# google-deepmind/meltingpot

Hardware: NVIDIA H100
Metric: env_steps_per_sec (higher is better)
Workload: dtype u8

## Files before the change

meltingpot_b200/build.py:

```python

from __future__ import annotations

import os
import shutil
import subprocess

_HERE = os.path.dirname(os.path.abspath(__file__))
SOURCES = ['engine.cu']
HEADERS = ['common.cuh', 'family_load.h', 'render.cuh', 'step_common.cuh', 'step_clean_up.cuh', 'step_commons.cuh', 'step_territory.cuh', 'step_coins.cuh', 'step_mining.cuh', 'state_bank.cuh']
LIB_PATH = os.path.join(_HERE, 'libmpengine.so')

NVCC_FLAGS = [
    '-gencode', 'arch=compute_90a,code=sm_90a', '-lineinfo', '-O3',
    '-std=c++17', '--fmad=false', '-shared', '-Xcompiler', '-fPIC',
]


def _nvcc() -> str:
  for cand in (shutil.which('nvcc'), '/usr/local/cuda/bin/nvcc'):
    if cand and os.path.exists(cand):
      return cand
  raise FileNotFoundError('nvcc not found')


def is_stale() -> bool:
  if not os.path.exists(LIB_PATH):
    return True
  built = os.path.getmtime(LIB_PATH)
  deps = [os.path.join(_HERE, 'csrc', f) for f in SOURCES + HEADERS]
  root = os.path.dirname(_HERE)
  deps += [os.path.join(root, 'include', 'mp_engine.h'),
           os.path.join(root, 'include', 'mpb_format.h')]
  return any(os.path.getmtime(d) > built for d in deps if os.path.exists(d))


def build(force: bool = False, verbose: bool = False) -> str:
  if not force and not is_stale():
    return LIB_PATH
  cmd = [_nvcc()] + NVCC_FLAGS
  if verbose:
    cmd += ['-Xptxas', '-v']
  cmd += ['-o', LIB_PATH] + [os.path.join(_HERE, 'csrc', s) for s in SOURCES]
  subprocess.check_call(cmd)
  return LIB_PATH


if __name__ == '__main__':
  print(build(force=True, verbose=True))
```

meltingpot_b200/csrc/engine.cu:

```cuda
#include <cuda_runtime.h>

#include <algorithm>
#include <cstdio>
#include <cstring>
#include <map>
#include <string>
#include <variant>
#include <vector>

#include "../../include/mp_engine.h"
#include "../../include/mpb_format.h"
#include "common.cuh"
#include "family_load.h"
#include "render.cuh"
#include "step_clean_up.cuh"
#include "step_commons.cuh"
#include "step_territory.cuh"
#include "step_coins.cuh"
#include "step_mining.cuh"
#include "state_bank.cuh"

static_assert(MP_MAX_ROUTE_CHOICES == MP_ROUTE_CHOICES && MP_MAX_ROUTE_PLAYERS == MP_MAX_PLAYERS,
              "mp_route_draw's table is DrawnActions'");
namespace {
// ... 825 lines not shown
  RecordLayout& R = E->record;
  R = RecordLayout{};
  uint32_t off = 16;
  int rc = MP_OK;
  auto row = [&](void* base, uint32_t bytes, uint32_t align) {
    if (R.n_rows == MP_RECORD_MAX_ROWS) { rc = fail(MP_E_UNSUPPORTED, "more than %d per-env state arrays", MP_RECORD_MAX_ROWS); return; }
    off = (off + align - 1) / align * align;
    R.row[R.n_rows++] = {static_cast<uint8_t*>(base), bytes, bytes, off};
    off += bytes;
  };
  auto own = [&](auto*& p, uint32_t bytes, uint32_t align = 16) {
    if (allocate && !rc) rc = E->alloc((size_t)E->B * bytes / sizeof *p, &p);
    row(p, bytes, align);
  };
  own(S.key, 8, 8);
  row(E->variants.active, 1, 1); row(E->variants.pending, 1, 1);
  own(S.grid, T.L * T.cells_pad * 2); own(S.avatar, P * 16); own(S.av_timer, P * 16);
  own(S.apple, T.nA_pad); own(S.dirt, T.nD_pad); own(S.water, T.nW_pad); own(S.apple_count, T.nA_pad);
  own(S.fam_u8, S.fam_u8_stride); own(S.fam_u16, S.fam_u16_stride * 2); own(S.av_extra, P * 32);
  own(S.packed, (P + 2) * 8); own(S.env, ENV_COLS * 4);
  row(S.reward, P * 8, 16); row(S.discount, 8, 16); row(S.step_type, 8, 16);
  for (int k = 0; k < T.n_scalar; ++k) row(S.scalar_obs + (size_t)k * E->B * P, P * 8, 16);
  own(S.events, S.max_events * 12); own(S.n_events, 4);
  if (rc) return rc;
  R.record_bytes = (off + 15) / 16 * 16;
  const uint64_t h = E->blob_hash;
  R.tag = make_uint4(kRecordFormat, (uint32_t)R.record_bytes, (uint32_t)h, (uint32_t)(h >> 32));
  CUDA_TRY(cudaMemcpy(E->d_record_layout, &R, sizeof R, cudaMemcpyHostToDevice));
  return MP_OK;
}

}

extern "C" {

const char* mp_last_error(void) { return g_error.c_str(); }
const char* mp_version(void) { return "meltingpot_b200 engine 0.1 (sm_90a)"; }

}

namespace {
int setup_variants(Decoded& D, const void* const* blobs, const size_t* blob_bytes, int n);
int upload_tables(mp_engine* E, Decoded& D);
int upload_variants(mp_engine* E, const Decoded& D, const void* const* blobs, const size_t* blob_bytes, int n, const uint8_t* env_variant_host);

int create(const void* const* blobs, const size_t* blob_sizes, int n_blobs, const uint8_t* env_variant, int num_envs, int device,
           uint64_t seed, uint64_t env_index_base, uint32_t flags, mp_handle* out) {
  Decoded D(n_blobs);
  int rc = build_tables(D, blobs, blob_sizes, n_blobs, flags);
  if (rc == MP_OK && n_blobs > 1) rc = setup_variants(D, blobs, blob_sizes, n_blobs);
  if (rc != MP_OK) return rc;
  int n_dev = 0;
  cudaError_t e = cudaGetDeviceCount(&n_dev);
  if (e != cudaSuccess || n_dev == 0) return fail(MP_E_NO_DEVICE, "no CUDA device available (%s); this engine has no CPU path", cudaGetErrorString(e));
  if (device < 0 || device >= n_dev || device >= MP_MAX_DEVICES) return fail(MP_E_INVALID, "device %d out of range (0..%d)", device, n_dev - 1);
  cudaDeviceProp prop;
  CUDA_TRY(cudaGetDeviceProperties(&prop, device));
  if (prop.major != 9 || prop.minor != 0) return fail(MP_E_NO_DEVICE, "device %d is sm_%d%d; kernels are built for sm_90a only", device, prop.major, prop.minor);
  DeviceGuard guard(device);
  mp_engine* E = new mp_engine();
  clear_last_launch(E);
  E->device = device; E->B = num_envs; E->flags = flags; E->sm_count = prop.multiProcessorCount;
  E->blob_hash = fnv1a(blobs[0], blob_sizes[0]);
  rc = upload_tables(E, D);
  if (rc == MP_OK && n_blobs > 1) rc = upload_variants(E, D, blobs, blob_sizes, n_blobs, env_variant);
  if (rc == MP_OK) rc = build_plan(E);
  if (rc != MP_OK) {
    const std::string msg = g_error;
    mp_destroy(E);
    g_error = msg;
    return rc;
  }
  const Tables& T = E->T;
  State& S = E->S;
  S.B = num_envs; E->key_base = seed + env_index_base;
  const size_t B = num_envs, P = T.P;
  {
    S.max_events = round_up(std::max(MP_MIN_EVENTS, T.P * (3 * D.beam_cells + 4 + T.P)), 16);
  }
  S.fam_u8_stride = std::max(16, RU_COUNT * T.nR_pad); S.fam_u16_stride = std::max(16, RS_COUNT * T.nR_pad);
  E->scalar_block_bytes = (B * P + B + B + std::max<size_t>(1, T.n_scalar) * B * P) * 8;
  if ((rc = E->alloc(E->scalar_block_bytes, &E->scalar_block)) || (rc = E->alloc(B * P * E->R.player_bytes, &S.rgb)) ||
      (rc = E->alloc(B * (size_t)E->R.world_bytes, &S.world_rgb)) || (rc = E->alloc(B * P, &E->d_actions)) ||
      (rc = E->alloc(1, &E->d_record_layout))) {
    mp_destroy(E);
    return rc;
  }
  S.reward = reinterpret_cast<double*>(E->scalar_block);
  S.discount = S.reward + B * P;
  S.step_type = reinterpret_cast<int64_t*>(S.discount + B);
  S.scalar_obs = reinterpret_cast<double*>(S.step_type + B);
  if ((rc = layout_state(E, true))) {
    mp_destroy(E);
    return rc;
  }
  S.rgb_env_stride = P * E->R.player_bytes; S.world_env_stride = E->R.world_bytes;
  {
    std::vector<int32_t> env0(B * ENV_COLS, 0);
    for (size_t b = 0; b < B; ++b) { env0[b * ENV_COLS + ENV_EPISODE] = -1; env0[b * ENV_COLS + ENV_DONE] = 1; }
    std::vector<uint64_t> key0(B);
    for (size_t b = 0; b < B; ++b) key0[b] = E->key_base + b;
    cudaError_t ce = cudaMemcpy(S.env, env0.data(), env0.size() * sizeof(int32_t), cudaMemcpyHostToDevice);
    if (ce == cudaSuccess) ce = cudaMemcpy(S.key, key0.data(), key0.size() * sizeof(uint64_t), cudaMemcpyHostToDevice);
    if (ce != cudaSuccess) { mp_destroy(E); return fail(MP_E_CUDA, "cudaMemcpy(env / key) failed: %s", cudaGetErrorString(ce)); }
  }
  E->step_smem = E->family->step_smem(T, n_blobs > 1);
  {
    const int ncp = (E->R.view_w + 3) / 4, ncw = (T.W + (32 >> E->R.wstrip_log2) - 1) / (32 >> E->R.wstrip_log2);
#define MP_RENDER_INST(NCP, NCW)                                                                                  \
  {                                                                                                               \
    E->render_fns[RENDER_PLAIN] = k_render<NCP, NCW, RENDER_PLAIN>;                                               \
    E->render_fns[RENDER_GATHER] = k_render<NCP, NCW, RENDER_GATHER>;                                             \
    E->render_fns[RENDER_ROUTED] = k_render<NCP, NCW, RENDER_ROUTED>; E->inst_ncp = NCP; E->inst_ncw = NCW;       \
  }
    if (ncp <= 3 && ncw <= 3) MP_RENDER_INST(3, 3)
    else if (ncp <= 3 && ncw <= 4) MP_RENDER_INST(3, 4)
    else if (ncp <= 3 && ncw <= 5) MP_RENDER_INST(3, 5)
    else if (ncp <= 4 && ncw <= 5) MP_RENDER_INST(4, 5)
#undef MP_RENDER_INST
    else { mp_destroy(E); return fail(MP_E_UNSUPPORTED, "view of %d cells / map of %d cells wide (max 16 / 40)", E->R.view_w, T.W); }
    const int wrows = 1 << E->R.wstrip_log2;
    if (flags & MP_FLAG_DEBUG_PLAIN_LANE_MAP) {
      for (int l = 0; l < 32; ++l) { E->R.pmap[l] = 0; for (int i = 0; i < 4; ++i) E->R.pmap[l] |= (uint32_t)std::min(63, (l >> 3) + 4 * i) << (6 * i); }
      for (int l = 0; l < 32; ++l) { E->R.wmap[l] = 0; for (int i = 0; i < 5; ++i) E->R.wmap[l] |= (uint32_t)std::min(63, (l >> E->R.wstrip_log2) + (32 >> E->R.wstrip_log2) * i) << (6 * i); }
    } else if ((flags & MP_FLAG_DEBUG_SCATTER_LANE_MAP) && make_lane_map(8, E->R.view_w, 3 * E->R.view_w, ncp, E->R.pmap) &&
               make_lane_map(wrows, T.W, 3 * T.W, ncw, E->R.wmap)) {
      E->lane_map_players = E->lane_map_world = 2;
    } else {
      E->lane_map_players = 1 + 16 * make_lane_map_cells(8, E->R.view_w, 3 * E->R.view_w, ncp, E->R.pmap);
      E->lane_map_world = 1 + 16 * make_lane_map_cells(wrows, T.W, 3 * T.W, ncw, E->R.wmap);
    }
  }
  cudaError_t ce = cudaSuccess;
  for (auto fn : E->render_fns)
    if (ce == cudaSuccess) ce = cudaFuncSetAttribute(fn, cudaFuncAttributeMaxDynamicSharedMemorySize, kRenderSmemLimit);
  {
    static int step_smem_max[MP_MAX_DEVICES] = {};
    const int need = (int)E->step_smem;
    if (ce == cudaSuccess && need > 48 * 1024 && need > step_smem_max[device]) {
      for (const FamilyEntry& f : kFamilies)
        for (const auto& by_restore : f.step)
          for (const auto& by_actions : by_restore)
            for (const void* k : by_actions)
              if (ce == cudaSuccess) ce = cudaFuncSetAttribute(k, cudaFuncAttributeMaxDynamicSharedMemorySize, need);
      if (ce == cudaSuccess) step_smem_max[device] = need;
    }
  }
  if (ce != cudaSuccess) { mp_destroy(E); return fail(MP_E_CUDA, "cudaFuncSetAttribute failed: %s", cudaGetErrorString(ce)); }
  mp_buffers& bf = E->buffers;
  bf.num_envs = num_envs; bf.num_players = T.P; bf.rgb_h = E->R.view_h * 8; bf.rgb_w = E->R.view_w * 8;
  bf.world_h = T.H * 8; bf.world_w = T.W * 8; bf.num_actions = T.n_actions; bf.num_scalar_obs = T.n_scalar;
  bf.rgb = S.rgb; bf.world_rgb = S.world_rgb; bf.reward = S.reward; bf.discount = S.discount; bf.step_type = S.step_type;
  bf.scalar_obs = S.scalar_obs; bf.avatar_state = S.avatar; bf.grid = S.grid; bf.timestep_packed = S.packed;
  bf.grid_layers = T.L; bf.grid_cells = T.cells; bf.grid_cells_padded = T.cells_pad;
  bf.events = S.events; bf.event_count = S.n_events; bf.max_events = S.max_events;
  bf.scalar_block = E->scalar_block; bf.scalar_block_bytes = E->scalar_block_bytes;
  E->render_bytes = (uint64_t)P * E->R.player_bytes + (uint64_t)E->R.world_bytes + (uint64_t)T.L * T.cells * 2;
  E->algo_bytes = (uint64_t)P * E->R.player_bytes + (uint64_t)E->R.world_bytes + 8ull * ((1 + T.n_scalar) * P + 2) + 8ull * P + 2ull * T.L * T.cells * 2;
  *out = E;
  return MP_OK;
}

int same_sections(const void* b0, size_t n0, const void* bv, size_t nv, const char* const* map_sections,
                  const char* const* sprite_sections) {
  const bool maps = map_sections != nullptr;
  const MpbHeader* h0 = static_cast<const MpbHeader*>(b0);
  const MpbHeader* hv = static_cast<const MpbHeader*>(bv);
// ... 812 lines not shown
  if (!rc) rc = check_extents(h, ext, "mp_state_restore");
  if (rc) return rc;
  cudaStream_t st = (cudaStream_t)stream;
  k_state_restore<<<(h->B + 7) / 8, 256, 0, st>>>(h->record, slot_of_env, static_cast<const uint8_t*>(bank), n_slots, h->B,
                                                  (flags & MP_RESTORE_REKEY) ? 1 : 0, h->key_base);
  ++h->launches;
  CUDA_TRY(cudaGetLastError());
  clear_last_launch(h);
  return launch_render(h, st);
}

int mp_run(mp_handle h, const mp_request* r, void* stream) {
  if (!h || !r) return fail(MP_E_INVALID, "mp_run: null handle or request");
  DeviceGuard guard(h->device);
  int rc = check_call(h, *r);
  if (rc) return rc;
  const StepRestore restore{h->d_record_layout, r->slot_of_env, static_cast<const uint8_t*>(r->bank), r->n_slots,
                            (r->restore_flags & MP_RESTORE_REKEY) ? 1 : 0, h->key_base};
  const mp_player_actions* a = r->player_actions;
  RowActions rows{};
  if (a) rows = {a->row_of_player, reinterpret_cast<const uint8_t*>(a->action), a->action_row_stride, a->n_rows};
  DrawnActions drawn{};
  if (r->draw) {
    const mp_route_draw& d = *r->draw;
    drawn.row_of_player = d.row_of_player; drawn.action = rows.action; drawn.stride = rows.stride;
    drawn.n_rows = d.n_rows;
    memcpy(drawn.n_choices, d.n_choices, sizeof drawn.n_choices);
    memcpy(drawn.base, d.row_base, sizeof drawn.base);
    memcpy(drawn.per_env, d.rows_per_env, sizeof drawn.per_env);
  }
  const cudaStream_t st = (cudaStream_t)stream;
  const bool render_follows = r->reset || r->out || r->players;
  if ((rc = launch_state(h, r->actions, r->env_mask, r->reset ? 1 : 0, st, render_follows, r->bank ? &restore : nullptr,
                         a ? &rows : nullptr, r->draw ? &drawn : nullptr)))
    return rc;
  return launch_render(h, st, r->out, r->players);
}

int mp_launch_count(mp_handle h, uint64_t* out) {
  if (!h || !out) return fail(MP_E_INVALID, "null argument");
  *out = h->launches;
  return MP_OK;
}

int mp_debug_render_plan(mp_handle h, int32_t out[MP_RENDER_PLAN_FIELDS]) {
  if (!h || !out) return fail(MP_E_INVALID, "mp_debug_render_plan: null argument");
  const RenderPlan& R = h->R;
  const int32_t v[MP_RENDER_PLAN_FIELDS] = {R.n_teams, R.team_threads, R.wstrip_log2, R.smem_bytes, R.n_total, R.rec_stride, R.stage_bytes,
                                            R.grid_bytes, h->lane_map_players, h->lane_map_world, h->inst_ncp, h->inst_ncw};
  memcpy(out, v, sizeof v);
  return MP_OK;
}

int mp_debug_last_launch(mp_handle h, int32_t out[MP_LAST_LAUNCH_FIELDS]) {
  if (!h || !out) return fail(MP_E_INVALID, "mp_debug_last_launch: null argument");
  memcpy(out, h->last_launch, sizeof h->last_launch);
  return MP_OK;
}

int mp_debug_render_tables(mp_handle h, int32_t* n_total, uint8_t* pair, uint8_t* flags) {
  if (!h) return fail(MP_E_INVALID, "null handle");
  if (n_total) *n_total = h->n_total;
  if (pair) memcpy(pair, h->host_pair.data(), h->host_pair.size());
  if (flags) memcpy(flags, h->host_sflags.data(), h->host_sflags.size());
  return MP_OK;
}

int mp_debug_observations(mp_handle h, int32_t* position, int32_t* orientation, int32_t* layer, int32_t* zap_matrix, void* stream) {
  if (!h) return fail(MP_E_INVALID, "null handle");
  DeviceGuard guard(h->device);
  k_debug_obs<<<h->B, 128, 0, (cudaStream_t)stream>>>(h->T, h->S, position, orientation, layer, zap_matrix, h->R.view_w, h->R.view_h);
  ++h->launches;
  CUDA_TRY(cudaGetLastError());
  return MP_OK;
}

int mp_debug_lane_map(int n_rows, int n_cells, int pitch_slots, int iters, int scattered, uint32_t out[32]) {
  if (!out || (n_rows != 8 && n_rows != 4 && n_rows != 2) || n_cells < 1 || n_cells > 62 || iters < 1 || iters > 5) return fail(MP_E_INVALID, "mp_debug_lane_map: bad arguments");
  if (!scattered) { if (n_cells > (32 / n_rows) * iters) return fail(MP_E_INVALID, "mp_debug_lane_map: too few turns"); make_lane_map_cells(n_rows, n_cells, pitch_slots, iters, out); return MP_OK; }
  if (!make_lane_map(n_rows, n_cells, pitch_slots, iters, out)) return fail(MP_E_UNSUPPORTED, "no conflict-free dealing for %d rows x %d cells in %d turns", n_rows, n_cells, iters);
  return MP_OK;
}

int mp_algorithmic_bytes(mp_handle h, uint64_t* per_env_step, uint64_t* render_per_env_step) {
  if (!h) return fail(MP_E_INVALID, "null handle");
  if (per_env_step) *per_env_step = h->algo_bytes;
  if (render_per_env_step) *render_per_env_step = h->render_bytes;
  return MP_OK;
}

}
```

meltingpot_b200/csrc/render.cuh:

```cuda
#pragma once

#include <cstdio>

#include "common.cuh"

#define RENDER_MAX_TEAMS 4
#define RENDER_MAX_THREADS 1024
#ifndef TEAM_THREADS
#define TEAM_THREADS 512
#endif
#ifndef RENDER_SLOTS
#define RENDER_SLOTS 1
#endif

struct RenderPlan {
  int view_w, view_h;
  int player_bytes;
  int world_bytes;
  int grid_bytes;
  int atlas_bytes;
  int n_total;
  int rec_stride;
  uint32_t magic_view_h;
  int off_atlas, off_pair, off_map, off_team0, team_stride;
  int toff_grid, toff_rec, toff_stage;
  int wstrip_log2;
  int stage_bytes;
  int smem_bytes;
  int team_threads;
  int n_teams;
  int n_player_items, n_items;
  int prow_bytes, wrow_bytes;
  int pitem_bytes, witem_bytes;
  int h_oob, h_oov;
  int h_empty;
  uint32_t pmap[32], wmap[32];
};

__device__ __forceinline__ uint32_t smem_u32(const void* p) { return (uint32_t)__cvta_generic_to_shared(p); }

__device__ __forceinline__ void mbar_init(uint64_t* bar, int count) {
  asm volatile("mbarrier.init.shared::cta.b64 [%0], %1;" ::"r"(smem_u32(bar)), "r"(count));
}
__device__ __forceinline__ void mbar_expect_tx(uint64_t* bar, uint32_t bytes) {
  asm volatile("mbarrier.arrive.expect_tx.shared::cta.b64 _, [%0], %1;" ::"r"(smem_u32(bar)), "r"(bytes) : "memory");
}
__device__ __forceinline__ void mbar_wait(uint64_t* bar, uint32_t parity) {
  asm volatile(
      "{\n"
      ".reg .pred p;\n"
      "WAIT_%=:\n"
      "mbarrier.try_wait.parity.shared::cta.b64 p, [%0], %1;\n"
      "@p bra DONE_%=;\n"
      "bra WAIT_%=;\n"
      "DONE_%=:\n"
      "}\n" ::"r"(smem_u32(bar)), "r"(parity) : "memory");
}
__device__ __forceinline__ void bulk_load(void* dst_smem, const void* src_gmem, uint32_t bytes, uint64_t* bar) {
  asm volatile("cp.async.bulk.shared::cluster.global.mbarrier::complete_tx::bytes [%0], [%1], %2, [%3];" ::"r"(smem_u32(dst_smem)),
               "l"(src_gmem), "r"(bytes), "r"(smem_u32(bar))
               : "memory");
}
__device__ __forceinline__ uint64_t make_evict_first_policy() {
  uint64_t policy;
  asm volatile("createpolicy.fractional.L2::evict_first.b64 %0, 1.0;" : "=l"(policy));
  return policy;
}
__device__ __forceinline__ void bulk_store(void* dst_gmem, const void* src_smem, uint32_t bytes, uint64_t policy) {
  asm volatile("cp.async.bulk.global.shared::cta.bulk_group.L2::cache_hint [%0], [%1], %2, %3;" ::"l"(dst_gmem), "r"(smem_u32(src_smem)),
               "r"(bytes), "l"(policy)
               : "memory");
  asm volatile("cp.async.bulk.commit_group;" ::: "memory");
}
template <int N>
__device__ __forceinline__ void bulk_wait_read() {
  asm volatile("cp.async.bulk.wait_group.read %0;" ::"n"(N) : "memory");
}
__device__ __forceinline__ void fence_async_smem() { asm volatile("fence.proxy.async.shared::cta;" ::: "memory"); }
__device__ __forceinline__ void group_sync(int bar_id, int threads) { asm volatile("bar.sync %0, %1;" ::"r"(bar_id), "r"(threads) : "memory"); }

__device__ __forceinline__ uint32_t blend_px(uint32_t dst, uint32_t src) {
  const uint32_t a = src >> 24;
  const uint32_t ia = 255u - a;
  uint32_t rb = (src & 0x00FF00FFu) * a + (dst & 0x00FF00FFu) * ia;
  uint32_t g = ((src >> 8) & 0xFFu) * a + ((dst >> 8) & 0xFFu) * ia;
  rb += 0x00010001u; rb += (rb >> 8) & 0x00FF00FFu; rb = (rb >> 8) & 0x00FF00FFu;
  g += 1u; g += g >> 8; g = (g >> 8) & 0xFFu;
  return rb | (g << 8);
}

#define ENT_SHIFT 13
#define ENT_VALUE 0x1fff
#define ENT_OPAQUE 0x2000
#define ENT_REMAP 0x4000
#define ENT_BINARY 0x8000

__device__ __forceinline__ uint32_t select_px(uint32_t dst, uint32_t src) { return (int32_t)src < 0 ? src : dst; }

__device__ __forceinline__ void compose_row(uint32_t px[8], const uint8_t* __restrict__ s_atlas, const uint16_t* __restrict__ rec,
                                            const int16_t* __restrict__ s_map, int viewer_orient, int py) {
  const int n = rec[0];
#pragma unroll
  for (int k = 0; k < 8; ++k) px[k] = 0;
  for (int k = 1; k <= n; ++k) {
    const uint32_t e = rec[k];
    int sprite = (e & ENT_VALUE) >> 2;
    if (e & ENT_REMAP) sprite = s_map[sprite];
    const int facing = ((int)(e & 3) - viewer_orient) & 3;
    const uint8_t* t = s_atlas + (sprite * 4 + facing) * 256 + py * 16;
    const uint4 lo = *reinterpret_cast<const uint4*>(t);
    const uint4 hi = *reinterpret_cast<const uint4*>(t + 128);
    if (e & ENT_BINARY) {
      px[0] = select_px(px[0], lo.x); px[1] = select_px(px[1], lo.y); px[2] = select_px(px[2], lo.z); px[3] = select_px(px[3], lo.w);
      px[4] = select_px(px[4], hi.x); px[5] = select_px(px[5], hi.y); px[6] = select_px(px[6], hi.z); px[7] = select_px(px[7], hi.w);
    } else {
      px[0] = blend_px(px[0], lo.x); px[1] = blend_px(px[1], lo.y); px[2] = blend_px(px[2], lo.z); px[3] = blend_px(px[3], lo.w);
      px[4] = blend_px(px[4], hi.x); px[5] = blend_px(px[5], hi.y); px[6] = blend_px(px[6], hi.z); px[7] = blend_px(px[7], hi.w);
    }
  }
}

#define REC_FAST 0x8000

template <int LMAX>
__device__ __forceinline__ void cell_pass(const Tables& T, const RenderPlan& R, const uint16_t* __restrict__ s_grid, uint16_t* __restrict__ s_rec,
                                          const uint8_t* __restrict__ s_flags, const uint8_t* __restrict__ s_pair, int gtid, int gthreads, uint32_t dbg) {
  for (int c = gtid; c < T.cells; c += gthreads) {
    uint32_t v[LMAX];
#pragma unroll
    for (int l = 0; l < LMAX; ++l) v[l] = l < T.L ? s_grid[l * T.cells_pad + c] : 0u;
    uint32_t nz = 0, oq = 0;
#pragma unroll
    for (int l = 0; l < LMAX; ++l) {
      const uint32_t f = v[l] ? s_flags[(v[l] - 1) >> 2] : 8u;
      nz |= ((f & 8u) ? 0u : 1u) << l;
      oq |= (f & 1u) << l;
    }
    oq &= ~1u;
    const int lo = oq ? 31 - __clz(oq) : 0;
    uint32_t cand = nz & (0xffffffffu << lo);
    uint16_t* r = s_rec + c * R.rec_stride;
    int n = 0;
    uint32_t cur = 0, cf = 0;
    bool merging = true;
    while (cand) {
      const int l = __ffs(cand) - 1;
      cand &= cand - 1;
      const uint32_t vl = s_grid[l * T.cells_pad + c];
      if (cur == 0) { cur = vl; cf = s_flags[(vl - 1) >> 2]; continue; }
      if (merging) {
        const uint32_t m = s_pair[((cur - 1) >> 2) * R.n_total + ((vl - 1) >> 2)];
        if (m && (((cur - 1) ^ (vl - 1)) & 3u) == 0) { cur = 1 + m * 4 + ((vl - 1) & 3u); cf = 5; continue; }
        merging = false;
      }
      r[1 + n++] = (uint16_t)((cur - 1) | (cf << ENT_SHIFT));
      cur = vl; cf = s_flags[(vl - 1) >> 2];
    }
    if (cur) r[1 + n++] = (uint16_t)((cur - 1) | (cf << ENT_SHIFT));
    if ((n == 1 && (cf & 1u)) || ((dbg & 256u) && cur)) r[0] = (uint16_t)(REC_FAST | (cur - 1));
    else r[0] = n ? (uint16_t)n : (uint16_t)R.h_empty;
  }
}

__device__ __forceinline__ void store_row(uint8_t* dst, const uint32_t px[8]) {
  uint2 a, b, c;
  a.x = __byte_perm(px[0], px[1], 0x4210); a.y = __byte_perm(px[1], px[2], 0x5421);
  b.x = __byte_perm(px[2], px[3], 0x6542); b.y = __byte_perm(px[4], px[5], 0x4210);
  c.x = __byte_perm(px[5], px[6], 0x5421); c.y = __byte_perm(px[6], px[7], 0x6542);
  uint2* d = reinterpret_cast<uint2*>(dst);
  d[0] = a; d[1] = b; d[2] = c;
}

__device__ __forceinline__ void fast_row(uint32_t px[8], const uint8_t* __restrict__ s_atlas, int h, int py) {
  const uint8_t* t = s_atlas + (h & 0x7fff) * 256 + py * 16;
  const uint4 lo = *reinterpret_cast<const uint4*>(t);
  const uint4 hi = *reinterpret_cast<const uint4*>(t + 128);
  px[0] = lo.x; px[1] = lo.y; px[2] = lo.z; px[3] = lo.w; px[4] = hi.x; px[5] = hi.y; px[6] = hi.z; px[7] = hi.w;
}

struct ViewerInfo {
  int ax, ay, ao, alive, fdx, fdy, rdx, rdy;
};

enum { RENDER_PLAIN = 0, RENDER_GATHER = 1, RENDER_ROUTED = 2 };
template <int NCP, int NCW, int MODE>
__global__ void __launch_bounds__(RENDER_MAX_THREADS, 1) k_render(Tables T, State S, RenderPlan R, uint32_t flags,
                                                            const __grid_constant__ RowSegments G) {
  constexpr bool GATHER = MODE == RENDER_GATHER, ROUTED = MODE == RENDER_ROUTED;
  extern __shared__ __align__(128) uint8_t smem[];
  uint64_t* bar = reinterpret_cast<uint64_t*>(smem);
  uint8_t* s_atlas = smem + R.off_atlas;
  const uint8_t* s_pair = smem + R.off_pair;
  int16_t* s_map = reinterpret_cast<int16_t*>(smem + R.off_map);
  __shared__ uint8_t s_opaque[256];
  __shared__ ViewerInfo s_view_all[RENDER_MAX_TEAMS][MP_MAX_PLAYERS];
  __shared__ int s_next_item[RENDER_MAX_TEAMS];
  __shared__ uint8_t s_players_all[RENDER_MAX_TEAMS][MP_MAX_PLAYERS];
  __shared__ int s_route_all[RENDER_MAX_TEAMS][3];

  const int tid = threadIdx.x;
  int team = 0;
#pragma unroll
  for (int k = 1; k < RENDER_MAX_TEAMS; ++k) team += tid >= k * R.team_threads;
  asm volatile("" : "+r"(team));
  const int ttid = tid - team * R.team_threads;
  const int lane = tid & 31, twarp = ttid >> 5;
  uint8_t* s_team = smem + R.off_team0 + team * R.team_stride;
  uint16_t* s_grid = reinterpret_cast<uint16_t*>(s_team + R.toff_grid);
  uint16_t* s_rec = reinterpret_cast<uint16_t*>(s_team + R.toff_rec);
  uint8_t* s_stage = s_team + R.toff_stage + twarp * R.stage_bytes;
  ViewerInfo* s_view = s_view_all[team];
  uint8_t* s_players = s_players_all[team];
  int* s_route = s_route_all[team];
  uint64_t* gbar = &bar[1 + team];

  const int n_streams = gridDim.x * R.n_teams;
  const int rounds = S.B / n_streams;
  const int tail0 = rounds * n_streams;
  const int n_tail = (S.B - tail0 - (int)blockIdx.x + (int)gridDim.x - 1) / (int)gridDim.x;
  const int n_iters = rounds + (n_tail > 0 ? n_tail : 0);
  const int first = blockIdx.x * R.n_teams + team;
  if (tid == 0) {
    for (int i = 0; i < 1 + R.n_teams; ++i) mbar_init(&bar[i], 1);
    asm volatile("fence.mbarrier_init.release.cluster;" ::: "memory");
  }
  if (ttid == 0) s_next_item[team] = 0;
  asm volatile("griddepcontrol.launch_dependents;" ::: "memory");
  __syncthreads();
  if (tid == 0) {
    mbar_expect_tx(&bar[0], (uint32_t)R.atlas_bytes);
    bulk_load(s_atlas, T.atlas, (uint32_t)R.atlas_bytes, &bar[0]);
  }
  for (int i = tid; i < (T.P + 1) * R.n_total; i += (int)blockDim.x) s_map[i] = T.sprite_map[i];
  for (int i = tid; i < R.n_total; i += (int)blockDim.x) s_opaque[i] = T.sprite_opaque[i];
  for (int i = tid; i < R.n_total * R.n_total; i += (int)blockDim.x) smem[R.off_pair + i] = T.sprite_pair[i];
  asm volatile("griddepcontrol.wait;" ::: "memory");
  if (GATHER && tid == 64 && S.g_step > 1ull) {
    for (int r = 0; r < S.g_world; ++r)
      while (*(const volatile unsigned long long*)(S.g_flags + r) + 1ull < S.g_step) __nanosleep(200);
  }
  if (ttid == 0 && rounds > 0) {
    mbar_expect_tx(gbar, (uint32_t)R.grid_bytes);
    bulk_load(s_grid, S.grid + (size_t)first * T.L * T.cells_pad, (uint32_t)R.grid_bytes, gbar);
  }
  __syncthreads();
  mbar_wait(&bar[0], 0);

  const int wlog = R.wstrip_log2, wrows = 1 << wlog;
  const int slot_bytes = R.stage_bytes / RENDER_SLOTS;
  const uint64_t store_policy = make_evict_first_policy();
  uint32_t pcells = R.pmap[lane], wcells = R.wmap[lane];
  asm volatile("" : "+r"(pcells), "+r"(wcells));
  uint32_t slot = 0;
  int gtid = ttid, gthreads = R.team_threads, bar_id = 1 + team;
  int* next_ctr = &s_next_item[team];
  for (int it = 0; it < n_iters; ++it) {
    if (it == rounds) {
      __syncthreads();
      uint8_t* s_team0 = smem + R.off_team0;
      s_grid = reinterpret_cast<uint16_t*>(s_team0 + R.toff_grid);
      s_rec = reinterpret_cast<uint16_t*>(s_team0 + R.toff_rec);
      s_view = s_view_all[0];
      s_players = s_players_all[0]; s_route = s_route_all[0];
      gbar = &bar[1];
      next_ctr = &s_next_item[0];
      gtid = tid; gthreads = (int)blockDim.x; bar_id = 0;
      if (tid == 0) {
        mbar_expect_tx(gbar, (uint32_t)R.grid_bytes);
        bulk_load(s_grid, S.grid + (size_t)(tail0 + (int)blockIdx.x) * T.L * T.cells_pad, (uint32_t)R.grid_bytes, gbar);
      }
    }
    const int b = it < rounds ? first + it * n_streams : tail0 + (int)blockIdx.x + (it - rounds) * (int)gridDim.x;
    if (gtid < T.P) {
      const int4 a = *reinterpret_cast<const int4*>(S.avatar + ((size_t)b * T.P + gtid) * 4);
      ViewerInfo vi;
      vi.ax = a.x; vi.ay = a.y; vi.ao = a.z; vi.alive = a.w;
      vi.fdx = dir_dx(a.z); vi.fdy = dir_dy(a.z); vi.rdx = dir_dx((a.z + 1) & 3); vi.rdy = dir_dy((a.z + 1) & 3);
      s_view[gtid] = vi;
    }
    if (ROUTED && gtid < 32) {
      bool on = gtid < T.P;
      if (on && G.s[0].rgb) on = row_segment(G, S.pr.row_of_player[(size_t)b * T.P + gtid]) >= 0;
      const uint32_t m = __ballot_sync(MP_FULL, on);
      if (on) s_players[__popc(m & ((1u << gtid) - 1u))] = (uint8_t)gtid;
      if (gtid == 0) {
        s_route[0] = G.s[0].rgb ? __popc(m) * R.view_h : R.n_player_items;
        int wrow = 0, wn = R.n_items - R.n_player_items;
        if (S.pr.world_rgb) {
          wrow = S.pr.world_row_of_env[b];
          if ((uint32_t)wrow >= (uint32_t)S.pr.world_n_rows) wn = 0;
        }
        s_route[1] = wn; s_route[2] = wrow;
      }
    }
    mbar_wait(gbar, (uint32_t)(it & 1));
    if (!(flags & 64u) || it == 0) {
      if (T.L <= 8) cell_pass<8>(T, R, s_grid, s_rec, s_opaque, s_pair, gtid, gthreads, flags);
      else if (T.L <= 10) cell_pass<10>(T, R, s_grid, s_rec, s_opaque, s_pair, gtid, gthreads, flags);
      else if (T.L <= 12) cell_pass<12>(T, R, s_grid, s_rec, s_opaque, s_pair, gtid, gthreads, flags);
      else cell_pass<MP_MAX_LAYERS>(T, R, s_grid, s_rec, s_opaque, s_pair, gtid, gthreads, flags);
    }
    group_sync(bar_id, gthreads);
    if (gtid == 0 && it + 1 < n_iters && it + 1 != rounds) {
      const int nb = it + 1 < rounds ? b + n_streams : b + (int)gridDim.x;
      mbar_expect_tx(gbar, (uint32_t)R.grid_bytes);
      bulk_load(s_grid, S.grid + (size_t)nb * T.L * T.cells_pad, (uint32_t)R.grid_bytes, gbar);
    }

    int next_item = 0;
    if (lane == 0) next_item = atomicAdd(next_ctr, 1);
    const int r_pitems = ROUTED ? s_route[0] : 0;
    for (;;) {
      const int item = __shfl_sync(MP_FULL, next_item, 0);
      if (ROUTED ? item - r_pitems >= s_route[1] : item >= R.n_items) break;
      if (lane == 0) next_item = atomicAdd(next_ctr, 1);
      uint8_t* buf = s_stage + (slot % RENDER_SLOTS) * slot_bytes;
      ++slot;
      if (lane == 0) bulk_wait_read<RENDER_SLOTS - 1>();
      __syncwarp();
      if (item < (ROUTED ? r_pitems : R.n_player_items)) {
        const int k = (int)(((uint32_t)item * R.magic_view_h) >> 16), cy = item - k * R.view_h;
        const int p = ROUTED ? (int)s_players[k] : k;
        const ViewerInfo vi = s_view[p];
        const int16_t* map = s_map + p * R.n_total;
        const int py = lane & 7;
        const int df = T.view_f - cy;
        const int bx = vi.ax + vi.fdx * df - vi.rdx * T.view_l, by = vi.ay + vi.fdy * df - vi.rdy * T.view_l;
        int hdr[NCP];
        if (!(flags & 16u)) {
        int myh = R.h_oov;
        if (lane < R.view_w && vi.alive) {
          int wx = bx + vi.rdx * lane, wy = by + vi.rdy * lane;
          if (wrap_or_reject(T, wx, wy)) {
            const int cell = wy * T.W + wx, h = s_rec[cell * R.rec_stride];
            myh = (h & REC_FAST) ? ((h & ~3) | ((h - vi.ao) & 3)) : cell;
          } else {
            myh = R.h_oob;
          }
        }
#pragma unroll
        for (int i = 0; i < NCP; ++i) hdr[i] = __shfl_sync(MP_FULL, myh, (pcells >> (6 * i)) & 31);
#pragma unroll
        for (int i = 0; i < NCP; ++i) {
          const int cx = (pcells >> (6 * i)) & 63;
          uint32_t q[8];
          fast_row(q, s_atlas, (hdr[i] & REC_FAST) ? hdr[i] : 0, py);
          if (!(hdr[i] & REC_FAST)) compose_row(q, s_atlas, s_rec + hdr[i] * R.rec_stride, map, vi.ao, py);
          if (cx < R.view_w) store_row(buf + py * R.prow_bytes + cx * 24, q);
        }
        }
        if (!(flags & 128u)) fence_async_smem();
        __syncwarp();
        if (lane == 0 && !(flags & 32u)) {
          const size_t in_env = (size_t)p * R.player_bytes + (size_t)cy * R.pitem_bytes;
          if (ROUTED && G.s[0].rgb) {
            const int row = S.pr.row_of_player[(size_t)b * T.P + p];
            const RowSegment& g = G.s[row_segment(G, row)];
            bulk_store(g.rgb + (size_t)(row - g.row_begin) * g.rgb_row_stride + (size_t)cy * R.pitem_bytes, buf, (uint32_t)R.pitem_bytes, store_policy);
          }
          else bulk_store(S.rgb + b * S.rgb_env_stride + in_env, buf, (uint32_t)R.pitem_bytes, store_policy);
          if (GATHER) {
            const size_t off = (size_t)b * T.P * R.player_bytes + in_env;
            for (int r = 0; r < S.g_world; ++r) bulk_store(S.g_rgb[r] + off, buf, (uint32_t)R.pitem_bytes, store_policy);
          }
        }
      } else {
        const int wi = item - (ROUTED ? r_pitems : R.n_player_items), wy = wi >> (3 - wlog);
        const int py = ((wi & ((8 >> wlog) - 1)) << wlog) | (lane & (wrows - 1));
        const int16_t* map = s_map + T.P * R.n_total;
        const uint16_t* rowrec = s_rec + wy * T.W * R.rec_stride;
        int hdr[NCW];
        if (!(flags & 16u)) {
#pragma unroll
        for (int i = 0; i < NCW; ++i) {
          const int cx = (wcells >> (6 * i)) & 63;
          hdr[i] = cx < T.W ? (int)rowrec[cx * R.rec_stride] : R.h_oov;
        }
#pragma unroll
        for (int i = 0; i < NCW; ++i) {
          const int cx = (wcells >> (6 * i)) & 63;
          uint32_t q[8];
          fast_row(q, s_atlas, (hdr[i] & REC_FAST) ? hdr[i] : 0, py);
          if (!(hdr[i] & REC_FAST)) compose_row(q, s_atlas, rowrec + min(cx, T.W - 1) * R.rec_stride, map, 0, py);
          if (cx < T.W) store_row(buf + (py & (wrows - 1)) * R.wrow_bytes + cx * 24, q);
        }
        }
        if (!(flags & 128u)) fence_async_smem();
        __syncwarp();
        if (lane == 0 && !(flags & 32u)) {
          const size_t in_env = (size_t)wi * R.witem_bytes;
          if (ROUTED && S.pr.world_rgb)
            bulk_store(S.pr.world_rgb + (size_t)s_route[2] * S.pr.world_rgb_row_stride + in_env, buf, (uint32_t)R.witem_bytes, store_policy);
          else bulk_store(S.world_rgb + b * S.world_env_stride + in_env, buf, (uint32_t)R.witem_bytes, store_policy);
          if (GATHER) {
            const size_t off = (size_t)b * R.world_bytes + in_env;
            for (int r = 0; r < S.g_world; ++r) bulk_store(S.g_wrgb[r] + off, buf, (uint32_t)R.witem_bytes, store_policy);
          }
        }
      }
    }
    if (S.x_raise && it == 0) exchange_push(T, S);
    if (S.out.on && it == 0) deliver_scalars(T, S);
    if (ROUTED && S.pr.scalars_on && it == 0) deliver_player_scalars(T, S, G);
    group_sync(bar_id, gthreads);
    if (gtid == 0) *next_ctr = 0;
  }
  if (lane == 0) { if (GATHER) asm volatile("cp.async.bulk.wait_group 0;" ::: "memory"); else bulk_wait_read<0>(); }
}
```

Before: 8.856 million.

## Deal render envs dynamically via global atomic counters instead of static striding

Replaces the static round-robin assignment of environments to render teams with a global atomic work queue. Teams claim envs as they finish, and the tail envs are claimed through a second counter and rendered by the whole CTA. The last CTA resets the counters for the next launch. This is meant to fix load imbalance between teams and CTAs, at the cost of global atomics and extra __syncthreads; it also adds an optional timeline-instrumented build.

New measurement: 8.984 million, median of 6. 1.5% higher.

```diff
diff --git a/meltingpot_b200/build.py b/meltingpot_b200/build.py
--- a/meltingpot_b200/build.py
+++ b/meltingpot_b200/build.py
@@ -9,6 +9,7 @@
 SOURCES = ['engine.cu']
 HEADERS = ['common.cuh', 'family_load.h', 'render.cuh', 'step_common.cuh', 'step_clean_up.cuh', 'step_commons.cuh', 'step_territory.cuh', 'step_coins.cuh', 'step_mining.cuh', 'state_bank.cuh']
 LIB_PATH = os.path.join(_HERE, 'libmpengine.so')
+TIMELINE_LIB_PATH = os.path.join(_HERE, 'libmpengine_timeline.so')
 
 NVCC_FLAGS = [
     '-gencode', 'arch=compute_90a,code=sm_90a', '-lineinfo', '-O3',
@@ -24,9 +25,9 @@
 
 
 def is_stale() -> bool:
-  if not os.path.exists(LIB_PATH):
+  if not os.path.exists(LIB_PATH) or not os.path.exists(TIMELINE_LIB_PATH):
     return True
-  built = os.path.getmtime(LIB_PATH)
+  built = min(os.path.getmtime(LIB_PATH), os.path.getmtime(TIMELINE_LIB_PATH))
   deps = [os.path.join(_HERE, 'csrc', f) for f in SOURCES + HEADERS]
   root = os.path.dirname(_HERE)
   deps += [os.path.join(root, 'include', 'mp_engine.h'),
@@ -37,11 +38,16 @@
 def build(force: bool = False, verbose: bool = False) -> str:
   if not force and not is_stale():
     return LIB_PATH
-  cmd = [_nvcc()] + NVCC_FLAGS
-  if verbose:
-    cmd += ['-Xptxas', '-v']
-  cmd += ['-o', LIB_PATH] + [os.path.join(_HERE, 'csrc', s) for s in SOURCES]
-  subprocess.check_call(cmd)
+  srcs = [os.path.join(_HERE, 'csrc', s) for s in SOURCES]
+  cmd = [_nvcc()] + NVCC_FLAGS + (['-Xptxas', '-v'] if verbose else []) + ['-o', LIB_PATH] + srcs
+  tl_cmd = [_nvcc()] + NVCC_FLAGS + ['-DMP_RENDER_TIMELINE', '-o', TIMELINE_LIB_PATH] + srcs
+  tl = subprocess.Popen(tl_cmd, stdout=subprocess.PIPE, stderr=subprocess.STDOUT)
+  try:
+    subprocess.check_call(cmd)
+  finally:
+    tl_out = tl.communicate()[0]
+  if tl.returncode:
+    raise subprocess.CalledProcessError(tl.returncode, tl_cmd, tl_out)
   return LIB_PATH
 
 
diff --git a/meltingpot_b200/csrc/engine.cu b/meltingpot_b200/csrc/engine.cu
--- a/meltingpot_b200/csrc/engine.cu
+++ b/meltingpot_b200/csrc/engine.cu
@@ -931,7 +931,7 @@
   E->scalar_block_bytes = (B * P + B + B + std::max<size_t>(1, T.n_scalar) * B * P) * 8;
   if ((rc = E->alloc(E->scalar_block_bytes, &E->scalar_block)) || (rc = E->alloc(B * P * E->R.player_bytes, &S.rgb)) ||
       (rc = E->alloc(B * (size_t)E->R.world_bytes, &S.world_rgb)) || (rc = E->alloc(B * P, &E->d_actions)) ||
-      (rc = E->alloc(1, &E->d_record_layout))) {
+      (rc = E->alloc(1, &E->d_record_layout)) || (rc = E->alloc(RENDER_DEAL_WORDS, &E->R.deal))) {
     mp_destroy(E);
     return rc;
   }
@@ -1910,6 +1910,30 @@
   return MP_OK;
 }
 
+#ifdef MP_RENDER_TIMELINE
+int mp_debug_render_timeline(mp_handle h, int reset, int32_t dims[4], uint64_t* stamps, uint64_t* globaltimes, uint32_t* strips) {
+  if (!h) return fail(MP_E_INVALID, "null handle");
+  DeviceGuard guard(h->device);
+  if (dims) { dims[0] = TL_CTAS; dims[1] = RENDER_MAX_TEAMS; dims[2] = TL_ITERS; dims[3] = TL_STAMPS; }
+  CUDA_TRY(cudaDeviceSynchronize());
+  void *p_stamp, *p_global, *p_strips;
+  CUDA_TRY(cudaGetSymbolAddress(&p_stamp, g_tl_stamp));
+  CUDA_TRY(cudaGetSymbolAddress(&p_global, g_tl_global));
+  CUDA_TRY(cudaGetSymbolAddress(&p_strips, g_tl_strips));
+  if (reset) {
+    CUDA_TRY(cudaMemset(p_stamp, 0xff, sizeof g_tl_stamp));
+    CUDA_TRY(cudaMemset(p_global, 0, sizeof g_tl_global));
+    CUDA_TRY(cudaMemset(p_strips, 0, sizeof g_tl_strips));
+  } else {
+    if (stamps) CUDA_TRY(cudaMemcpy(stamps, p_stamp, sizeof g_tl_stamp, cudaMemcpyDeviceToHost));
+    if (globaltimes) CUDA_TRY(cudaMemcpy(globaltimes, p_global, sizeof g_tl_global, cudaMemcpyDeviceToHost));
+    if (strips) CUDA_TRY(cudaMemcpy(strips, p_strips, sizeof g_tl_strips, cudaMemcpyDeviceToHost));
+  }
+  CUDA_TRY(cudaDeviceSynchronize());
+  return MP_OK;
+}
+#endif
+
 int mp_algorithmic_bytes(mp_handle h, uint64_t* per_env_step, uint64_t* render_per_env_step) {
   if (!h) return fail(MP_E_INVALID, "null handle");
   if (per_env_step) *per_env_step = h->algo_bytes;
diff --git a/meltingpot_b200/csrc/render.cuh b/meltingpot_b200/csrc/render.cuh
--- a/meltingpot_b200/csrc/render.cuh
+++ b/meltingpot_b200/csrc/render.cuh
@@ -35,7 +35,9 @@
   int h_oob, h_oov;
   int h_empty;
   uint32_t pmap[32], wmap[32];
+  unsigned int* deal;
 };
+#define RENDER_DEAL_WORDS 4
 
 __device__ __forceinline__ uint32_t smem_u32(const void* p) { return (uint32_t)__cvta_generic_to_shared(p); }
 
@@ -178,9 +180,36 @@
   px[0] = lo.x; px[1] = lo.y; px[2] = lo.z; px[3] = lo.w; px[4] = hi.x; px[5] = hi.y; px[6] = hi.z; px[7] = hi.w;
 }
 
+__device__ __forceinline__ int deal_env(unsigned int* ctr, int n) {
+  const int e = (int)atomicAdd(ctr, 1u);
+  return e < n ? e : -1;
+}
+
 struct ViewerInfo {
   int ax, ay, ao, alive, fdx, fdy, rdx, rdy;
 };
+
+#ifdef MP_RENDER_TIMELINE
+#define TL_CTAS 256
+#define TL_ITERS 64
+enum { TL_GRID_READY = 0, TL_RECORDS_DONE = 1, TL_LAST_CLAIMED = 2, TL_ENV_DONE = 3, TL_ENV = 4, TL_STAMPS = 5 };
+#define TL_TAIL 0x80000000u
+__device__ unsigned long long g_tl_stamp[TL_CTAS][RENDER_MAX_TEAMS][TL_ITERS][TL_STAMPS];
+__device__ unsigned long long g_tl_global[TL_CTAS][4];
+__device__ unsigned int g_tl_strips[TL_CTAS][RENDER_MAX_TEAMS];
+__device__ __forceinline__ unsigned long long tl_globaltimer() {
+  unsigned long long t;
+  asm volatile("mov.u64 %0, %%globaltimer;" : "=l"(t));
+  return t;
+}
+#define TL_STAMP(it, k) do { if (blockIdx.x < TL_CTAS && (it) < TL_ITERS) g_tl_stamp[blockIdx.x][team][it][k] = clock64(); } while (0)
+#define TL_STAMP_MIN(it, k) do { if (blockIdx.x < TL_CTAS && (it) < TL_ITERS) atomicMin(&g_tl_stamp[blockIdx.x][team][it][k], (unsigned long long)clock64()); } while (0)
+#define TL_COUNT_STRIP() do { if (blockIdx.x < TL_CTAS) atomicAdd(&g_tl_strips[blockIdx.x][team], 1u); } while (0)
+#else
+#define TL_STAMP(it, k) do {} while (0)
+#define TL_STAMP_MIN(it, k) do {} while (0)
+#define TL_COUNT_STRIP() do {} while (0)
+#endif
 
 enum { RENDER_PLAIN = 0, RENDER_GATHER = 1, RENDER_ROUTED = 2 };
 template <int NCP, int NCW, int MODE>
@@ -194,7 +223,7 @@
   int16_t* s_map = reinterpret_cast<int16_t*>(smem + R.off_map);
   __shared__ uint8_t s_opaque[256];
   __shared__ ViewerInfo s_view_all[RENDER_MAX_TEAMS][MP_MAX_PLAYERS];
-  __shared__ int s_next_item[RENDER_MAX_TEAMS];
+  __shared__ int s_deal[RENDER_MAX_TEAMS + 1][2];
   __shared__ uint8_t s_players_all[RENDER_MAX_TEAMS][MP_MAX_PLAYERS];
   __shared__ int s_route_all[RENDER_MAX_TEAMS][3];
 
@@ -215,17 +244,17 @@
   uint64_t* gbar = &bar[1 + team];
 
   const int n_streams = gridDim.x * R.n_teams;
-  const int rounds = S.B / n_streams;
-  const int tail0 = rounds * n_streams;
-  const int n_tail = (S.B - tail0 - (int)blockIdx.x + (int)gridDim.x - 1) / (int)gridDim.x;
-  const int n_iters = rounds + (n_tail > 0 ? n_tail : 0);
-  const int first = blockIdx.x * R.n_teams + team;
+  const int n_bal = S.B / n_streams * n_streams;
+  const int n_tail = S.B - n_bal;
   if (tid == 0) {
     for (int i = 0; i < 1 + R.n_teams; ++i) mbar_init(&bar[i], 1);
     asm volatile("fence.mbarrier_init.release.cluster;" ::: "memory");
   }
-  if (ttid == 0) s_next_item[team] = 0;
+  if (tid < 2 * (RENDER_MAX_TEAMS + 1)) (&s_deal[0][0])[tid] = 0;
   asm volatile("griddepcontrol.launch_dependents;" ::: "memory");
+#ifdef MP_RENDER_TIMELINE
+  if (tid == 0 && blockIdx.x < TL_CTAS) { g_tl_global[blockIdx.x][0] = tl_globaltimer(); g_tl_global[blockIdx.x][2] = clock64(); }
+#endif
   __syncthreads();
   if (tid == 0) {
     mbar_expect_tx(&bar[0], (uint32_t)R.atlas_bytes);
@@ -239,9 +268,14 @@
     for (int r = 0; r < S.g_world; ++r)
       while (*(const volatile unsigned long long*)(S.g_flags + r) + 1ull < S.g_step) __nanosleep(200);
   }
-  if (ttid == 0 && rounds > 0) {
-    mbar_expect_tx(gbar, (uint32_t)R.grid_bytes);
-    bulk_load(s_grid, S.grid + (size_t)first * T.L * T.cells_pad, (uint32_t)R.grid_bytes, gbar);
+  __syncthreads();
+  if (ttid == 0) {
+    const int e = deal_env(&R.deal[0], n_bal);
+    s_deal[team][1] = e;
+    if (e >= 0) {
+      mbar_expect_tx(gbar, (uint32_t)R.grid_bytes);
+      bulk_load(s_grid, S.grid + (size_t)e * T.L * T.cells_pad, (uint32_t)R.grid_bytes, gbar);
+    }
   }
   __syncthreads();
   mbar_wait(&bar[0], 0);
@@ -253,24 +287,34 @@
   asm volatile("" : "+r"(pcells), "+r"(wcells));
   uint32_t slot = 0;
   int gtid = ttid, gthreads = R.team_threads, bar_id = 1 + team;
-  int* next_ctr = &s_next_item[team];
-  for (int it = 0; it < n_iters; ++it) {
-    if (it == rounds) {
+  int* next_ctr = s_deal[team];
+  int ph = 0;
+  int it = 0;
+  for (;; ++it) {
+    int b = next_ctr[1];
+    if (b < 0) {
+      if (bar_id == 0) break;
+      int e = -1;
+      if (tid == 0) { e = deal_env(&R.deal[1], n_tail); s_deal[RENDER_MAX_TEAMS][1] = e < 0 ? -1 : n_bal + e; }
       __syncthreads();
       uint8_t* s_team0 = smem + R.off_team0;
       s_grid = reinterpret_cast<uint16_t*>(s_team0 + R.toff_grid);
       s_rec = reinterpret_cast<uint16_t*>(s_team0 + R.toff_rec);
       s_view = s_view_all[0];
       s_players = s_players_all[0]; s_route = s_route_all[0];
-      gbar = &bar[1];
-      next_ctr = &s_next_item[0];
+      gbar = &bar[0]; ph = 1;
+      next_ctr = s_deal[RENDER_MAX_TEAMS];
       gtid = tid; gthreads = (int)blockDim.x; bar_id = 0;
-      if (tid == 0) {
+      if (e >= 0) {
         mbar_expect_tx(gbar, (uint32_t)R.grid_bytes);
-        bulk_load(s_grid, S.grid + (size_t)(tail0 + (int)blockIdx.x) * T.L * T.cells_pad, (uint32_t)R.grid_bytes, gbar);
-      }
-    }
-    const int b = it < rounds ? first + it * n_streams : tail0 + (int)blockIdx.x + (it - rounds) * (int)gridDim.x;
+        bulk_load(s_grid, S.grid + (size_t)(n_bal + e) * T.L * T.cells_pad, (uint32_t)R.grid_bytes, gbar);
+      }
+      b = next_ctr[1];
+      if (b < 0) break;
+    }
+#ifdef MP_RENDER_TIMELINE
+    if (ttid == 0 && blockIdx.x < TL_CTAS && it < TL_ITERS) g_tl_stamp[blockIdx.x][team][it][TL_ENV] = (unsigned)b | (bar_id == 0 ? TL_TAIL : 0u);
+#endif
     if (gtid < T.P) {
       const int4 a = *reinterpret_cast<const int4*>(S.avatar + ((size_t)b * T.P + gtid) * 4);
       ViewerInfo vi;
@@ -293,18 +337,25 @@
         s_route[1] = wn; s_route[2] = wrow;
       }
     }
-    mbar_wait(gbar, (uint32_t)(it & 1));
-    if (!(flags & 64u) || it == 0) {
+    mbar_wait(gbar, (uint32_t)(ph & 1));
+    ++ph;
+    if (ttid == 0) TL_STAMP(it, TL_GRID_READY);
+    if (!(flags & 64u) || ph - (bar_id == 0) == 1) {
       if (T.L <= 8) cell_pass<8>(T, R, s_grid, s_rec, s_opaque, s_pair, gtid, gthreads, flags);
       else if (T.L <= 10) cell_pass<10>(T, R, s_grid, s_rec, s_opaque, s_pair, gtid, gthreads, flags);
       else if (T.L <= 12) cell_pass<12>(T, R, s_grid, s_rec, s_opaque, s_pair, gtid, gthreads, flags);
       else cell_pass<MP_MAX_LAYERS>(T, R, s_grid, s_rec, s_opaque, s_pair, gtid, gthreads, flags);
     }
     group_sync(bar_id, gthreads);
-    if (gtid == 0 && it + 1 < n_iters && it + 1 != rounds) {
-      const int nb = it + 1 < rounds ? b + n_streams : b + (int)gridDim.x;
-      mbar_expect_tx(gbar, (uint32_t)R.grid_bytes);
-      bulk_load(s_grid, S.grid + (size_t)nb * T.L * T.cells_pad, (uint32_t)R.grid_bytes, gbar);
+    if (ttid == 0) TL_STAMP(it, TL_RECORDS_DONE);
+    if (gtid == 0) {
+      const int e = bar_id == 0 ? deal_env(&R.deal[1], n_tail) : deal_env(&R.deal[0], n_bal);
+      const int nb = e < 0 ? -1 : (bar_id == 0 ? n_bal + e : e);
+      next_ctr[1] = nb;
+      if (nb >= 0) {
+        mbar_expect_tx(gbar, (uint32_t)R.grid_bytes);
+        bulk_load(s_grid, S.grid + (size_t)nb * T.L * T.cells_pad, (uint32_t)R.grid_bytes, gbar);
+      }
     }
 
     int next_item = 0;
@@ -312,7 +363,10 @@
     const int r_pitems = ROUTED ? s_route[0] : 0;
     for (;;) {
       const int item = __shfl_sync(MP_FULL, next_item, 0);
-      if (ROUTED ? item - r_pitems >= s_route[1] : item >= R.n_items) break;
+      if (ROUTED ? item - r_pitems >= s_route[1] : item >= R.n_items) {
+        if (lane == 0) TL_STAMP_MIN(it, TL_LAST_CLAIMED);
+        break;
+      }
       if (lane == 0) next_item = atomicAdd(next_ctr, 1);
       uint8_t* buf = s_stage + (slot % RENDER_SLOTS) * slot_bytes;
       ++slot;
@@ -352,6 +406,7 @@
         if (!(flags & 128u)) fence_async_smem();
         __syncwarp();
         if (lane == 0 && !(flags & 32u)) {
+          TL_COUNT_STRIP();
           const size_t in_env = (size_t)p * R.player_bytes + (size_t)cy * R.pitem_bytes;
           if (ROUTED && G.s[0].rgb) {
             const int row = S.pr.row_of_player[(size_t)b * T.P + p];
@@ -388,6 +443,7 @@
         if (!(flags & 128u)) fence_async_smem();
         __syncwarp();
         if (lane == 0 && !(flags & 32u)) {
+          TL_COUNT_STRIP();
           const size_t in_env = (size_t)wi * R.witem_bytes;
           if (ROUTED && S.pr.world_rgb)
             bulk_store(S.pr.world_rgb + (size_t)s_route[2] * S.pr.world_rgb_row_stride + in_env, buf, (uint32_t)R.witem_bytes, store_policy);
@@ -403,7 +459,20 @@
     if (S.out.on && it == 0) deliver_scalars(T, S);
     if (ROUTED && S.pr.scalars_on && it == 0) deliver_player_scalars(T, S, G);
     group_sync(bar_id, gthreads);
+    if (ttid == 0) TL_STAMP(it, TL_ENV_DONE);
     if (gtid == 0) *next_ctr = 0;
   }
+  if (it == 0) {
+    if (S.x_raise) exchange_push(T, S);
+    if (S.out.on) deliver_scalars(T, S);
+    if (ROUTED && S.pr.scalars_on) deliver_player_scalars(T, S, G);
+  }
+  if (tid == 0 && atomicAdd(&R.deal[2], 1u) == gridDim.x - 1) {
+    atomicExch(&R.deal[0], 0u); atomicExch(&R.deal[1], 0u); atomicExch(&R.deal[2], 0u);
+  }
   if (lane == 0) { if (GATHER) asm volatile("cp.async.bulk.wait_group 0;" ::: "memory"); else bulk_wait_read<0>(); }
-}
+#ifdef MP_RENDER_TIMELINE
+  __syncthreads();
+  if (tid == 0 && blockIdx.x < TL_CTAS) { g_tl_global[blockIdx.x][1] = tl_globaltimer(); g_tl_global[blockIdx.x][3] = clock64(); }
+#endif
+}
```
